# NVIDIA/tacotron2

Measured on AMD Instinct MI355X. Metric: mel-frames/sec (train fwd+bwd) LJSpeech hparams, higher is better.
Workload: dtype bf16; 1 GPU; BASELINE configs[1]: LJSpeech default hparams, batch_size=64/GPU, synthetic LJSpeech-shaped batches, full train step (fwd+loss+bwd+clip+Adam); global_batch=64, parallelism=dp1, optimizer=FusedAdam, compute=bf16 MFMA operands, f32 accumulate/state/master weights

## Files before the change

### include/tacotron2_amd.h

```cpp
#ifndef TACOTRON2_AMD_H
#define TACOTRON2_AMD_H

#include <stdint.h>

#ifdef __cplusplus
extern "C" {
#endif

#define T2AMD_ABI_VERSION 1
#define T2AMD_OK 0
#define T2AMD_ERR_ARG 1
#define T2AMD_ERR_LAUNCH 2

#define T2AMD_ATT_DIM 128
#define T2AMD_LOC_FILTERS 32
#define T2AMD_LOC_KERNEL 31
#define T2AMD_LOC_TAPS (2 * T2AMD_LOC_KERNEL)
#define T2AMD_ATT_SLICES 4

int t2amd_abi_version(void);
const char* t2amd_source_sha1(void);
const char* t2amd_last_error(void);
int t2amd_struct_sizes(int* out, int max_n);
int t2amd_set_validate_only(int on);
// ... 15 lines not shown
    long long strideSplitC;
    int accumulate;
    const float* bias;
    int act;
    const uint8_t* keep;
    long long ldkeep;
    float keep_scale;
    int convA_T, convA_C, convA_pad, convA_sign;
    int convB_T, convB_C, convB_pad;
    int precision;
} t2amd_gemm_desc;

int t2amd_gemm_tile_size(int M, int N, int precision, int nz, int a_kcontig, int b_kcontig);
int t2amd_gemm_f32(const t2amd_gemm_desc* d, void* stream);

int t2amd_splitk_reduce_f32(const float* partials, int nsplit, long long stride, float* out,
                            long long n, int accumulate, int perm_taps, int perm_ci, void* stream);
int t2amd_splitk_reduce2d_f32(const float* partials, int nsplit, long long stride, float* out, int rows, int cols,
                              long long ldo, int accumulate, void* stream);

typedef struct t2amd_gemm16_desc {
    const void* A;
    const void* B;
    float* C;
    int M, N, K;
    long long lda, ldb, ldc;
    int splitk;
    long long strideSplitC;
    int accumulate;
    const float* bias;
    int win_T, win_Tp;
} t2amd_gemm16_desc;
int t2amd_gemm16_tn(const t2amd_gemm16_desc* d, void* stream);
int t2amd_gemm16_kk(const t2amd_gemm16_desc* d, void* stream);
int t2amd_gemm16_kk_group(const t2amd_gemm16_desc* d, int count, void* stream);

int t2amd_cast_halo_bf16(const float* src, long long lds, void* dst, long long rows, int C, int T, int pad, void* stream);

int t2amd_pack_conv_bf16(const float* W, void* out, int Co, int Ci, int k, int Kp, int reversed, void* stream);

int t2amd_transpose_cast_bf16(const void* src, int src_is_bf16, long long lds, void* dst, long long ldd, int rows, int cols,
                              int rows_padded, void* stream);

int t2amd_bn_stats_f32(const float* x, long long ldx, int M, int N, double* ws, float* mean,
                       float* invstd, float* running_mean, float* running_var, float momentum,
                       float eps, void* stream);
int t2amd_bn_eval_invstd_f32(const float* running_var, float* invstd, int N, float eps, void* stream);
int t2amd_bn_act_fwd_f32(const float* x, long long ldx, float* y, long long ldy, int M, int N,
                         const float* mean, const float* invstd, const float* gamma,
                         const float* beta, int act, const uint8_t* keep, long long ldkeep,
                         float keep_scale, const int* lens, int row_valid_T, void* stream);
int t2amd_bn_act_fwd_img_f32(const float* x, long long ldx, float* y, long long ldy, int M, int N, const float* mean,
                             const float* invstd, const float* gamma, const float* beta, int act, const uint8_t* keep,
                             long long ldkeep, float keep_scale, void* y_img16, int T, int pad, void* stream);
int t2amd_bn_act_bwd_f32(float* dy, long long lddy, const float* y, long long ldy, const float* x,
                         long long ldx, int M, int N, const float* mean, const float* invstd,
                         const float* gamma, int act, const uint8_t* keep, long long ldkeep,
                         float keep_scale, double* ws, float* dgamma, float* dbeta, void* stream);
int t2amd_bn_act_bwd_img_f32(float* dy, long long lddy, const float* y, long long ldy, const float* x, long long ldx, int M, int N,
                             const float* mean, const float* invstd, const float* gamma, int act, const uint8_t* keep,
                             long long ldkeep, float keep_scale, double* ws, float* dgamma, float* dbeta, void* dx_img16, int T,
                             int pad, float* dbias, int keep_f32, void* stream);
int t2amd_colsum_f32(const float* x, long long ldx, int M, int N, double* ws, float* out,
                     int accumulate, void* stream);
int t2amd_colsum_bf16(const void* x16, long long ldx, int M, int N, double* ws, float* out, int accumulate, void* stream);

// ... 695 lines not shown
```

### tacotron2_amd/csrc/api.hip

```cpp
#include "common.h"
#include <string.h>
#include <vector>

static thread_local char g_err[512] = "";

extern "C" void t2amd_set_error_(const char* msg) {
    strncpy(g_err, msg ? msg : "", sizeof(g_err) - 1);
    g_err[sizeof(g_err) - 1] = 0;
}
extern "C" const char* t2amd_last_error(void) { return g_err; }
static int g_validate_only = 0;
extern "C" int t2amd_validate_only_flag_(void) { return g_validate_only; }
extern "C" int t2amd_set_validate_only(int on) { g_validate_only = on ? 1 : 0; return T2AMD_OK; }
extern "C" int t2amd_abi_version(void) { return T2AMD_ABI_VERSION; }
#ifndef T2AMD_SOURCE_SHA1
#define T2AMD_SOURCE_SHA1 ""
#endif
extern "C" const char* t2amd_source_sha1(void) { return T2AMD_SOURCE_SHA1; }

extern "C" int t2amd_struct_sizes(int* out, int max_n) {
    const int sizes[] = {
        (int)sizeof(t2amd_gemm_desc), (int)sizeof(t2amd_seg),       (int)sizeof(t2amd_lstm_step),
        (int)sizeof(t2amd_skinny_gemm), (int)sizeof(t2amd_addend),  (int)sizeof(t2amd_lstm_bwd),
        (int)sizeof(t2amd_attn_fwd),  (int)sizeof(t2amd_attn_bwd),  (int)sizeof(t2amd_dec_train),
        (int)sizeof(t2amd_dec_train_bwd), (int)sizeof(t2amd_lstm_seq), (int)sizeof(t2amd_dec_infer),
        (int)sizeof(t2amd_small_linear), (int)sizeof(t2amd_tensor_list), (int)sizeof(t2amd_adam_hyper),
        (int)sizeof(t2amd_dec_persist), (int)sizeof(t2amd_gemm16_desc),
    };
    const int n = (int)(sizeof(sizes) / sizeof(sizes[0]));
    for (int i = 0; i < n && i < max_n; ++i) out[i] = sizes[i];
    return n;
}

static int g_prof_tag = -1, g_prof_max = 0, g_prof_n = 0;
static std::vector<hipEvent_t> g_prof_ev;
static hipEvent_t g_cal_ev[8];
static int g_cal_have = 0, g_cal_done = 0;

extern "C" void t2amd_profile_mark_(int tag, int end, hipStream_t s) {
    if (g_prof_tag < 0 || tag != g_prof_tag || g_validate_only) return;
    if (!end) {
        if (g_prof_n >= g_prof_max) return;
        if (!g_cal_done) {
            if (!g_cal_have) {
                for (int i = 0; i < 8; ++i) (void)hipEventCreate(&g_cal_ev[i]);
                g_cal_have = 1;
// ... 518 lines not shown
```

### tacotron2_amd/csrc/common.h

```cpp
#pragma once
#include <hip/hip_runtime.h>
#include <hip/hip_ext.h>
#include <stdint.h>
#include <stdio.h>
#include "../../include/tacotron2_amd.h"

typedef float f32x4 __attribute__((ext_vector_type(4)));
typedef float f32x16 __attribute__((ext_vector_type(16)));

#define T2_WAVE 64

extern "C" void t2amd_set_error_(const char* msg);

#define T2_FAIL(msg)                                                                   \
    do {                                                                               \
        t2amd_set_error_(msg);                                                         \
        return T2AMD_ERR_ARG;                                                          \
    } while (0)

#define T2_REQUIRE(cond, msg)                                                          \
    do {                                                                               \
        if (!(cond)) T2_FAIL(msg);                                                     \
    } while (0)

extern "C" int t2amd_validate_only_flag_(void);

extern "C" void t2amd_profile_mark_(int tag, int end, hipStream_t s);

#define T2_LAUNCH(kern, grid, block, lds, stream, ...)                                 \
    do {                                                                               \
        if (!t2amd_validate_only_flag_())                                              \
            hipLaunchKernelGGL(kern, grid, block, lds, stream, __VA_ARGS__);           \
    } while (0)

extern "C" bool t2amd_profile_pair_(int tag, hipEvent_t* e0, hipEvent_t* e1);
#define T2_LAUNCH_ROLE(role, kern, grid, block, lds, stream, ...)                      \
    do {                                                                               \
        if (t2amd_validate_only_flag_()) break;                                        \
        hipEvent_t pe0_ = nullptr, pe1_ = nullptr;                                     \
        if (t2amd_profile_pair_(role, &pe0_, &pe1_))                                   \
            hipExtLaunchKernelGGL(kern, grid, block, lds, stream, pe0_, pe1_, 0, __VA_ARGS__); \
        else                                                                           \
            hipLaunchKernelGGL(kern, grid, block, lds, stream, __VA_ARGS__);           \
    } while (0)

#define T2_LAUNCH_CHECK()                                                              \
    do {                                                                               \
        if (t2amd_validate_only_flag_()) break;                                        \
        hipError_t e_ = hipGetLastError();                                             \
        if (e_ != hipSuccess) {                                                        \
            t2amd_set_error_(hipGetErrorString(e_));                                   \
            return T2AMD_ERR_LAUNCH;                                                   \
        }                                                                              \
    } while (0)

#define T2_PROPAGATE(call)                                                             \
    do {                                                                               \
        int rc_ = (call);                                                              \
// ... 158 lines not shown
```

### tacotron2_amd/csrc/gemm16.hip

```cpp
#include "common.h"
#include <stdlib.h>

typedef __bf16 g16_bf16x8 __attribute__((ext_vector_type(8)));
typedef __attribute__((address_space(3))) void* g16_lptr;
typedef __attribute__((address_space(1))) const void* g16_gptr;

#define G16_T 256
#define G16_BK 64
#define G16_IMG (G16_T * 128)
#define G16_NT 512

struct Gemm16Params {
    t2amd_gemm16_desc d;
    int ktiles_per_split;
};

struct G16Tile { int bx, by, bz; };
__device__ __forceinline__ G16Tile g16_tile_id() {
    const int nbx = gridDim.x, nby = gridDim.y;
    const int total = nbx * nby * (int)gridDim.z;
    const int L = blockIdx.x + nbx * (blockIdx.y + nby * blockIdx.z);
    const int xcd = L & 7, q = L >> 3;
    const int base = total >> 3, rem = total & 7;
    const int id = xcd * base + (xcd < rem ? xcd : rem) + q;
    const int per_z = nbx * nby;
    G16Tile t;
    t.bz = id / per_z;
    const int r = id - t.bz * per_z;
    const int G = 8;
    const int group = r / (G * nbx);
    const int first = group * G;
    const int gsz = (nby - first) < G ? (nby - first) : G;
    const int w = r - group * (G * nbx);
    t.by = first + w % gsz;
    t.bx = w / gsz;
    return t;
}

__global__ __launch_bounds__(G16_NT) void gemm16_tn_kernel(Gemm16Params p) {
    __shared__ __attribute__((aligned(16))) char smem[4 * G16_IMG];
    const t2amd_gemm16_desc& d = p.d;
    const int tid = threadIdx.x, lane = tid & 63;
    const int wave = __builtin_amdgcn_readfirstlane(tid >> 6);
    const int wm = wave >> 2, wn = wave & 3;
    const int l31 = lane & 31, lhi = lane >> 5;

    const G16Tile tile = g16_tile_id();
    const int split = tile.bz;
    const int row0 = tile.by * G16_T, col0 = tile.bx * G16_T;
    const int M = d.M, N = d.N;
    const int nkt_all = d.K / G16_BK;
    const int kt_beg = split * p.ktiles_per_split;
    int kt_end = kt_beg + p.ktiles_per_split;
    if (kt_end > nkt_all) kt_end = nkt_all;
    const int nk = kt_end > kt_beg ? kt_end - kt_beg : 0;

    const char* asrc[4];
    const char* bsrc[4];
    {
        const int rin = 8 * wave + (lane >> 3);
        const int chunk = (lane & 7) ^ ((rin >> 1) & 7);
#pragma unroll
        for (int i = 0; i < 4; ++i) {
            int ga = row0 + 64 * i + rin, gb = col0 + 64 * i + rin;
            ga = ga < M ? ga : M - 1;
            gb = gb < N ? gb : N - 1;
            asrc[i] = reinterpret_cast<const char*>(d.A) + ((long long)ga * d.lda + (long long)kt_beg * G16_BK) * 2 + chunk * 16;
            bsrc[i] = reinterpret_cast<const char*>(d.B) + ((long long)gb * d.ldb + (long long)kt_beg * G16_BK) * 2 + chunk * 16;
        }
    }
#define G16_ISSUE(STAGE)                                                                                         \
    {                                                                                                            \
        char* ad_ = smem + (STAGE) * G16_IMG + wave * 1024;                                                      \
        char* bd_ = smem + (2 + (STAGE)) * G16_IMG + wave * 1024;                                                \
        _Pragma("unroll") for (int i = 0; i < 4; ++i) {                                                          \
            __builtin_amdgcn_global_load_lds((g16_gptr)(asrc[i]), (g16_lptr)(ad_ + i * 8192), 16, 0, 0);         \
            __builtin_amdgcn_global_load_lds((g16_gptr)(bsrc[i]), (g16_lptr)(bd_ + i * 8192), 16, 0, 0);         \
            asrc[i] += 128; bsrc[i] += 128;                                                                      \
        }                                                                                                        \
    }

    unsigned aaddr[4][4], baddr[2][4];
    {
        const unsigned base = (unsigned)reinterpret_cast<size_t>((g16_lptr)(smem));
#pragma unroll
        for (int t = 0; t < 4; ++t) {
            const int r = wm * 128 + t * 32 + l31;
#pragma unroll
            for (int ks = 0; ks < 4; ++ks) aaddr[t][ks] = base + (unsigned)(r * 128 + (((2 * ks + lhi) ^ ((r >> 1) & 7)) << 4));
        }
#pragma unroll
        for (int t = 0; t < 2; ++t) {
            const int r = wn * 64 + t * 32 + l31;
#pragma unroll
            for (int ks = 0; ks < 4; ++ks)
                baddr[t][ks] = base + 2 * G16_IMG + (unsigned)(r * 128 + (((2 * ks + lhi) ^ ((r >> 1) & 7)) << 4));
        }
    }

    f32x16 acc[4][2];
#pragma unroll
    for (int i = 0; i < 4; ++i)
#pragma unroll
        for (int j = 0; j < 2; ++j)
#pragma unroll
            for (int r = 0; r < 16; ++r) acc[i][j][r] = 0.f;

    f32x4 fa[4], fb[2], ga[4], gb[2];
#define G16_READ(STAGE, KS, A_, B_)                                                                              \
    asm volatile(                                                                                                \
        "ds_read_b128 %0, %6 offset:%12\n\t"                                                                     \
        "ds_read_b128 %4, %10 offset:%12\n\t"                                                                    \
        "ds_read_b128 %1, %7 offset:%12\n\t"                                                                     \
        "ds_read_b128 %5, %11 offset:%12\n\t"                                                                    \
        "ds_read_b128 %2, %8 offset:%12\n\t"                                                                     \
        "ds_read_b128 %3, %9 offset:%12"                                                                         \
        : "=&v"(A_[0]), "=&v"(A_[1]), "=&v"(A_[2]), "=&v"(A_[3]), "=&v"(B_[0]), "=&v"(B_[1])                     \
        : "v"(aaddr[0][KS]), "v"(aaddr[1][KS]), "v"(aaddr[2][KS]), "v"(aaddr[3][KS]), "v"(baddr[0][KS]),          \
          "v"(baddr[1][KS]), "i"((STAGE) * G16_IMG)                                                              \
        : "memory");
#define G16_WAIT(A_, B_)                                                                                         \
    asm volatile("s_waitcnt lgkmcnt(0)"                                                                          \
                 : "+v"(A_[0]), "+v"(A_[1]), "+v"(A_[2]), "+v"(A_[3]), "+v"(B_[0]), "+v"(B_[1]) : : "memory");
#define G16_MFMA(A_, B_)                                                                                         \
    _Pragma("unroll") for (int i = 0; i < 4; ++i)                                                                \
        _Pragma("unroll") for (int j = 0; j < 2; ++j)                                                            \
            acc[i][j] = __builtin_amdgcn_mfma_f32_32x32x16_bf16(__builtin_bit_cast(g16_bf16x8, A_[i]),           \
                                                                __builtin_bit_cast(g16_bf16x8, B_[j]), acc[i][j], 0, 0, 0);
#define G16_TILE(STAGE)                                                                                          \
    {                                                                                                            \
        G16_READ(STAGE, 0, fa, fb) G16_WAIT(fa, fb)                                                              \
        G16_READ(STAGE, 1, ga, gb) __builtin_amdgcn_sched_barrier(0); G16_MFMA(fa, fb) __builtin_amdgcn_sched_barrier(0); G16_WAIT(ga, gb) \
        G16_READ(STAGE, 2, fa, fb) __builtin_amdgcn_sched_barrier(0); G16_MFMA(ga, gb) __builtin_amdgcn_sched_barrier(0); G16_WAIT(fa, fb) \
        G16_READ(STAGE, 3, ga, gb) __builtin_amdgcn_sched_barrier(0); G16_MFMA(fa, fb) __builtin_amdgcn_sched_barrier(0); G16_WAIT(ga, gb) \
        G16_MFMA(ga, gb)                                                                                         \
    }

    if (nk > 0) {
        G16_ISSUE(0)
        asm volatile("s_waitcnt vmcnt(0)" ::: "memory");
        __builtin_amdgcn_s_barrier();
        for (int kt = 0; kt + 1 < nk; kt += 2) {
            G16_ISSUE(1)
            G16_TILE(0)
            asm volatile("s_waitcnt vmcnt(0)" ::: "memory");
            __builtin_amdgcn_s_barrier();
            if (kt + 2 < nk) G16_ISSUE(0)
            G16_TILE(1)
            asm volatile("s_waitcnt vmcnt(0)" ::: "memory");
            __builtin_amdgcn_s_barrier();
        }
        if (nk & 1) G16_TILE(0)
    }
#undef G16_ISSUE
#undef G16_READ
#undef G16_WAIT
#undef G16_MFMA
#undef G16_TILE

    float* __restrict__ C = d.C + (long long)split * d.strideSplitC;
#pragma unroll
    for (int tm = 0; tm < 4; ++tm) {
#pragma unroll
        for (int tn = 0; tn < 2; ++tn) {
            const int gn = col0 + wn * 64 + tn * 32 + l31;
#pragma unroll
            for (int r = 0; r < 16; ++r) {
                const int gm = row0 + wm * 128 + tm * 32 + (r & 3) + 8 * (r >> 2) + 4 * lhi;
                long long crow = gm;
                bool live = gm < M;
                if (d.win_Tp > 0) {
                    const int b_ = gm / d.win_Tp, t_ = gm - b_ * d.win_Tp;
                    live = live && t_ < d.win_T;
                    crow = (long long)b_ * d.win_T + t_;
                }
                if (live && gn < N) {
                    float* cp = C + crow * d.ldc + gn;
                    float val = acc[tm][tn][r];
                    if (d.bias) val += d.bias[gn];
                    if (d.accumulate) val += *cp;
                    *cp = val;
                }
            }
        }
    }
}

extern "C" int t2amd_gemm16_tn(const t2amd_gemm16_desc* dp, void* stream) {
    T2_REQUIRE(dp != nullptr, "gemm16: null descriptor");
    Gemm16Params p;
    p.d = *dp;
    t2amd_gemm16_desc& d = p.d;
    T2_REQUIRE(d.A && d.B && d.C, "gemm16: null operand");
    T2_REQUIRE(d.M > 0 && d.N > 0 && d.K > 0 && d.K % G16_BK == 0, "gemm16: K must be a positive multiple of 64");
    T2_REQUIRE(t2_aligned16(d.A) && t2_aligned16(d.B) && d.lda % 8 == 0 && d.ldb % 8 == 0 && d.ldb >= d.K,
               "gemm16: operands must be 16-byte aligned with row strides that are multiples of 8 elements (B's >= K)");
    T2_REQUIRE(d.win_Tp == 0 || (d.win_T > 0 && d.win_T <= d.win_Tp && d.splitk == 1), "gemm16: bad window geometry");
    T2_REQUIRE(d.win_Tp > 0 || d.lda >= d.K, "gemm16: lda must be >= K unless the rows are windows");
    if (d.splitk < 1) d.splitk = 1;
    T2_REQUIRE(d.splitk == 1 || (!d.bias && !d.accumulate), "gemm16: split-K needs a plain epilogue");
    const int nkt = d.K / G16_BK;
    p.ktiles_per_split = t2_cdiv(nkt, d.splitk);
    dim3 grid(t2_cdiv(d.N, G16_T), t2_cdiv(d.M, G16_T), d.splitk);
    T2_REQUIRE(grid.y <= 65535 && grid.z <= 65535, "gemm16: grid too large");
    T2_LAUNCH(gemm16_tn_kernel, grid, dim3(G16_NT), 0, (hipStream_t)stream, p);
    T2_LAUNCH_CHECK();
    return T2AMD_OK;
}

typedef float g16_f32x2 __attribute__((ext_vector_type(2)));

#define G16_GROUP 4
struct Gemm16GroupParams {
    t2amd_gemm16_desc d[G16_GROUP];
    int coltile_end[G16_GROUP];
    int count;
};

__global__ __launch_bounds__(G16_NT) void gemm16_kk_kernel(Gemm16GroupParams p) {
    __shared__ __attribute__((aligned(16))) char smem[4 * G16_IMG];
    const int tid = threadIdx.x, lane = tid & 63;
    const int wave = __builtin_amdgcn_readfirstlane(tid >> 6);
    const int wm = wave >> 2, wn = wave & 3;
    const int l31 = lane & 31, lhi = lane >> 5;

    const G16Tile tile = g16_tile_id();
    const int split = tile.bz;
    int prob = 0;
#pragma unroll
    for (int j = 0; j + 1 < G16_GROUP; ++j)
        if (j + 1 < p.count && tile.bx >= p.coltile_end[j]) prob = j + 1;
    const int bx = tile.bx - (prob > 0 ? p.coltile_end[prob - 1] : 0);
    struct { const void* A; const void* B; float* C; int M, N, K; long long lda, ldb, ldc; long long strideSplitC; int accumulate;
             const float* bias; int splitk; } d;
    d.A = p.d[prob].A; d.B = p.d[prob].B; d.C = p.d[prob].C; d.M = p.d[prob].M; d.N = p.d[prob].N; d.K = p.d[prob].K;
    d.lda = p.d[prob].lda; d.ldb = p.d[prob].ldb; d.ldc = p.d[prob].ldc; d.strideSplitC = p.d[prob].strideSplitC;
    d.accumulate = p.d[prob].accumulate; d.bias = p.d[prob].bias; d.splitk = p.d[prob].splitk;
    const int row0 = tile.by * G16_T, col0 = bx * G16_T;
// ... 310 lines not shown
```

### tacotron2_amd/native.py

```python
import ctypes as C
import os

import torch

_HERE = os.path.dirname(os.path.abspath(__file__))
LIB_PATH = os.environ.get("T2AMD_LIB", os.path.join(_HERE, "lib", "libtacotron2_amd.so"))

TORCH_OPS_PATH = os.path.join(_HERE, "lib", "libtacotron2_amd_torch.so")

ATT_DIM = 128
LOC_FILTERS = 32
LOC_KERNEL = 31
LOC_TAPS = 62
ATT_SLICES = 4

_f32p = C.c_void_p
_i64 = C.c_longlong


class GemmDesc(C.Structure):
    _fields_ = [
        ("A", _f32p), ("B", _f32p), ("C", _f32p),
        ("M", C.c_int), ("N", C.c_int), ("K", C.c_int),
        ("lda", _i64), ("ldb", _i64), ("ldc", _i64),
# ... 195 lines not shown
class DecPersist(C.Structure):
    _fields_ = [
        ("Ti", C.c_int), ("E", C.c_int), ("H", C.c_int), ("P", C.c_int), ("C", C.c_int),
        ("max_steps", C.c_int), ("gate_threshold", C.c_float),
        ("Wa16", C.c_void_p), ("Wd16", C.c_void_p), ("bias_a", _f32p), ("bias_d", _f32p),
        ("Wq", _f32p), ("U", _f32p), ("v", _f32p), ("Wf", _f32p), ("bias_f", _f32p), ("W2", _f32p),
        ("memory", _f32p), ("pm", _f32p), ("keep_prenet", C.c_void_p),
        ("PG", _f32p), ("ALIGN", _f32p), ("out_length", C.c_void_p), ("status", C.c_void_p),
        ("steps_done", C.c_void_p), ("mailbox", C.c_void_p), ("trace", _f32p), ("timing", C.c_void_p),
        ("weights_f32", C.c_int),
    ]


PERSIST_TIMEOUT = 7
MAX_TENSORS = 64


class TensorList(C.Structure):
    _fields_ = [("param", C.c_void_p * MAX_TENSORS), ("grad", C.c_void_p * MAX_TENSORS),
                ("exp_avg", C.c_void_p * MAX_TENSORS), ("exp_avg_sq", C.c_void_p * MAX_TENSORS),
                ("numel", C.c_longlong * MAX_TENSORS), ("first_block", C.c_int * MAX_TENSORS), ("count", C.c_int)]


class AdamHyper(C.Structure):
    _fields_ = [("step_size", C.c_float), ("bc2_sqrt", C.c_float), ("one_minus_beta1", C.c_float),
                ("beta2", C.c_float), ("one_minus_beta2", C.c_float), ("eps", C.c_float), ("weight_decay", C.c_float)]


_STRUCTS = [GemmDesc, Seg, LstmStep, SkinnyGemm, Addend, LstmBwd, AttnFwd, AttnBwd, DecTrain,
            DecTrainBwd, LstmSeq, DecInfer, SmallLinear, TensorList, AdamHyper, DecPersist, Gemm16Desc]

SYMBOLS = [
    "t2amd_abi_version", "t2amd_source_sha1", "t2amd_last_error", "t2amd_struct_sizes", "t2amd_set_validate_only", "t2amd_profile_enable", "t2amd_profile_read", "t2amd_profile_event_overhead",
    "t2amd_gemm_f32", "t2amd_gemm_tile_size", "t2amd_splitk_reduce_f32", "t2amd_splitk_reduce2d_f32", "t2amd_gemm16_tn", "t2amd_gemm16_kk", "t2amd_gemm16_kk_group", "t2amd_transpose_cast_bf16", "t2amd_cast_halo_bf16", "t2amd_pack_conv_bf16",
    "t2amd_bn_stats_f32", "t2amd_bn_eval_invstd_f32", "t2amd_bn_act_fwd_f32", "t2amd_bn_act_bwd_f32", "t2amd_bn_act_bwd_img_f32", "t2amd_colsum_bf16", "t2amd_bn_act_fwd_img_f32",
    "t2amd_colsum_f32",
    "t2amd_embedding_fwd_f32", "t2amd_embedding_bwd_f32", "t2amd_philox_keep_mask", "t2amd_fill_f32",
    "t2amd_copy2d_f32", "t2amd_cast_bf16_f32", "t2amd_split_bf16x3_f32", "t2amd_transpose_f32", "t2amd_frames_to_time_major_f32",
    "t2amd_split_projection_f32", "t2amd_finalize_outputs_f32", "t2amd_grads_to_channel_last_f32",
    "t2amd_gather_dout_f32", "t2amd_relu_dropout_bwd_f32",
    "t2amd_lstm_step_fwd_f32", "t2amd_skinny_gemm_f32", "t2amd_lstm_pointwise_bwd_f32",
    "t2amd_lstm_step_fwd2_f32", "t2amd_skinny_gemm2_f32", "t2amd_lstm_pointwise_bwd2_f32",
    "t2amd_fold_location_f32", "t2amd_unfold_location_grads_f32",
    "t2amd_attention_step_fwd_f32", "t2amd_attention_step_bwd_f32",
    "t2amd_decoder_train_fwd_loop_f32", "t2amd_decoder_train_bwd_loop_f32",
    "t2amd_decoder_train_fwd_persistent_flag_bytes", "t2amd_decoder_train_fwd_persistent_supported", "t2amd_decoder_train_fwd_persistent_f32",
    "t2amd_lstm_seq_fwd_f32", "t2amd_lstm_seq_bwd_f32", "t2amd_decoder_infer_steps_f32",
    "t2amd_set_decoder_streams", "t2amd_set_bptt_cell_fold", "t2amd_get_bptt_cell_fold", "t2amd_attn_bwd_ws_floats",
    "t2amd_set_small_batch_max", "t2amd_get_small_batch_max", "t2amd_dec_infer_uses_tiles",
    "t2amd_set_attn_bwd_granules", "t2amd_attn_handoff_timeouts", "t2amd_set_attn_bwd_fused", "t2amd_attn_fwd_ws_floats", "t2amd_set_attn_fwd_fused", "t2amd_lstm_step_small_f32", "t2amd_linear_small_f32",
    "t2amd_lstm_seq_fwd2_f32", "t2amd_lstm_seq_bwd2_f32",
    "t2amd_lstm_seq_persistent_mailbox_bytes", "t2amd_lstm_seq_persistent_supported", "t2amd_lstm_seq_fwd2_persistent_f32",
    "t2amd_lstm_seq_batch_persistent_flag_bytes", "t2amd_lstm_seq_batch_persistent_supported", "t2amd_lstm_seq_fwd2_batch_persistent_f32", "t2amd_encoder_handoff_timeouts",
    "t2amd_lstm_seq_bwd2_batch_persistent_supported", "t2amd_lstm_seq_bwd2_batch_persistent_f32",
    "t2amd_reflect_pad_f32", "t2amd_reflect_index", "t2amd_stft_magnitude_f32", "t2amd_mel_log_compress_f32",
    "t2amd_mel_log_bwd_f32", "t2amd_stft_magnitude_bwd_f32", "t2amd_stft_frames_fold_f32", "t2amd_mel_l1_rows_per_slot",
    "t2amd_mel_l1_fwd_f32", "t2amd_mel_l1_bwd_f32",
    "t2amd_stft_loss_rows_per_slot", "t2amd_stft_loss_fwd_f32", "t2amd_stft_loss_finish_f64", "t2amd_stft_loss_bwd_f32",
    "t2amd_stft_loss_sum_f32",
    "t2amd_resample_plan", "t2amd_resample_fwd_f32", "t2amd_resample_bwd_f32",
    "t2amd_dtw_width", "t2amd_mel_cepstrum_f32", "t2amd_dtw_f32", "t2amd_dtw_backtrack",
    "t2amd_yin_plan", "t2amd_yin_f32",
    "t2amd_align_limits", "t2amd_align_workspace", "t2amd_monotonic_align_f32",
    "t2amd_forward_sum_workspace", "t2amd_forward_sum_f32", "t2amd_forward_sum_bwd_f32",
    "t2amd_aligner_workspace", "t2amd_aligner_pack_keys_f32", "t2amd_aligner_transpose_f32", "t2amd_aligner_rows_fwd_f32",
    "t2amd_aligner_rows_bwd_f32", "t2amd_aligner_scores_f32", "t2amd_aligner_scores_bwd_f32", "t2amd_aligner_product_f32",
    "t2amd_beta_binomial_log_prior_f32",
# ... 60 lines not shown
        "t2amd_skinny_gemm_f32": [pt(SkinnyGemm), _P],
        "t2amd_lstm_pointwise_bwd_f32": [pt(LstmBwd), _P],
        "t2amd_lstm_step_fwd2_f32": [pt(LstmStep), pt(LstmStep), _P],
        "t2amd_skinny_gemm2_f32": [pt(SkinnyGemm), pt(SkinnyGemm), _P],
        "t2amd_lstm_pointwise_bwd2_f32": [pt(LstmBwd), pt(LstmBwd), _P],
        "t2amd_fold_location_f32": [_P, _P, _P, _P],
        "t2amd_unfold_location_grads_f32": [_P, _P, _I, _P, _P, _P, _P, _P, _P],
        "t2amd_attention_step_fwd_f32": [pt(AttnFwd), _P],
        "t2amd_attention_step_bwd_f32": [pt(AttnBwd), _P],
        "t2amd_decoder_train_fwd_loop_f32": [pt(DecTrain), _P],
        "t2amd_decoder_train_fwd_persistent_flag_bytes": [_I, _I],
        "t2amd_decoder_train_fwd_persistent_supported": [pt(DecTrain), _I],
        "t2amd_decoder_train_fwd_persistent_f32": [pt(DecTrain), _P, _P, _P, _P],
        "t2amd_decoder_train_bwd_loop_f32": [pt(DecTrainBwd), _P],
        "t2amd_lstm_seq_fwd_f32": [pt(LstmSeq), _P],
        "t2amd_lstm_seq_bwd_f32": [pt(LstmSeq), _P],
        "t2amd_lstm_seq_fwd2_f32": [pt(LstmSeq), pt(LstmSeq), _P],
        "t2amd_lstm_seq_bwd2_f32": [pt(LstmSeq), pt(LstmSeq), _P],
        "t2amd_lstm_seq_persistent_mailbox_bytes": [_I, _I],
        "t2amd_lstm_seq_persistent_supported": [pt(LstmSeq)],
        "t2amd_lstm_seq_fwd2_persistent_f32": [pt(LstmSeq), pt(LstmSeq), _P, _P, _P],
        "t2amd_lstm_seq_batch_persistent_flag_bytes": [_I, _I, _I],
        "t2amd_lstm_seq_batch_persistent_supported": [pt(LstmSeq), _I, _I],
        "t2amd_lstm_seq_fwd2_batch_persistent_f32": [pt(LstmSeq), pt(LstmSeq), _P, _P, _P, _P],
        "t2amd_lstm_seq_bwd2_batch_persistent_supported": [pt(LstmSeq), _I, _I],
        "t2amd_lstm_seq_bwd2_batch_persistent_f32": [pt(LstmSeq), pt(LstmSeq), _P, _P, _P, _P],
        "t2amd_encoder_handoff_timeouts": [_I],
        "t2amd_decoder_infer_steps_f32": [pt(DecInfer), _P],
        "t2amd_struct_sizes": [pt(C.c_int), _I],
        "t2amd_set_validate_only": [_I],
        "t2amd_set_decoder_streams": [_I],
        "t2amd_set_bptt_cell_fold": [_I],
        "t2amd_get_bptt_cell_fold": [],
        "t2amd_set_small_batch_max": [_I],
        "t2amd_get_small_batch_max": [_I],
        "t2amd_dec_infer_uses_tiles": [_I, _I, _I, _I, _I, _I],
        "t2amd_attn_bwd_ws_floats": [_I, _I],
        "t2amd_set_attn_bwd_granules": [_I],
        "t2amd_attn_handoff_timeouts": [_I],
        "t2amd_set_attn_bwd_fused": [_I],
        "t2amd_attn_fwd_ws_floats": [_I, _I],
        "t2amd_set_attn_fwd_fused": [_I],
        "t2amd_lstm_step_small_f32": [pt(LstmStep), _P],
        "t2amd_linear_small_f32": [pt(SmallLinear), _P],
        "t2amd_profile_enable": [_I, _I],
        "t2amd_profile_read": [pt(C.c_float), pt(C.c_int)],
        "t2amd_profile_event_overhead": [pt(C.c_float)],
        "t2amd_reflect_pad_f32": [_P, _L, _P, _L, _I, _I, _I, _I, _P],
        "t2amd_stft_magnitude_f32": [_P, _L, _P, _L, _L, _I, _I, _P],
        "t2amd_mel_log_compress_f32": [_P, _L, _P, _I, _I, _I, _F, _P],
        "t2amd_mel_log_bwd_f32": [_P, _P, _L, _P, _L, _I, _I, _I, _F, _P],
        "t2amd_stft_magnitude_bwd_f32": [_P, _L, _P, _L, _P, _L, _L, _I, _I, _P],
        "t2amd_stft_frames_fold_f32": [_P, _L, _L, _P, _L, _L, _I, _I, _I, _I, _I, _I, _P],
        "t2amd_mel_l1_rows_per_slot": [_I],
        "t2amd_mel_l1_fwd_f32": [_P, _P, _P, _I, _I, _I, _I, _L, _P, _L, _P],
        "t2amd_mel_l1_bwd_f32": [_P, _P, _P, _P, _I, _I, _I, _I, _L, _P, _P],
        "t2amd_stft_loss_rows_per_slot": [_I],
        "t2amd_stft_loss_fwd_f32": [_P, _L, _P, _L, _P, _I, _I, _I, _F, _P, _L, _P],
        "t2amd_stft_loss_finish_f64": [_P, _L, _P, _P, _I, _F, _F, _P, _P, _P, _P],
        "t2amd_stft_loss_bwd_f32": [_P, _L, _P, _L, _P, _P, _P, _I, _I, _I, _I, _F, _P, _L, _L, _P],
        "t2amd_stft_loss_sum_f32": [_P, _L, _L, _I, _L, _P, _P],
        "t2amd_resample_plan": [_I, _I, _I, _I, pt(C.c_int), pt(C.c_int)],
        "t2amd_resample_fwd_f32": [_P, _L, _P, _I, _L, _P, _L, _L, _P, _P, _I, _I, _I, _I, _P],
        "t2amd_resample_bwd_f32": [_P, _L, _P, _I, _L, _L, _P, _L, _P, _P, _I, _I, _I, _I, _I, _P],
        "t2amd_dtw_width": [],
        "t2amd_mel_cepstrum_f32": [_P, _L, _L, _P, _I, _I, _I, _P, _I, _P, _P],
# ... 212 lines not shown
def tacotron2_loss_bwd(mel, post, tgt, gate, gate_tgt, upstream, d_mel, d_post, d_gate):
    for t in (mel, post, tgt, gate, gate_tgt, upstream, d_mel, d_post, d_gate):
        _fullc(t)
    _check(load().t2amd_tacotron2_loss_bwd_f32(ptr(mel), ptr(post), ptr(tgt), mel.numel(), ptr(gate), ptr(gate_tgt),
                                               gate.numel(), ptr(upstream), ptr(d_mel), ptr(d_post), ptr(d_gate), _stream()),
           "t2amd_tacotron2_loss_bwd_f32")


def loss_workspace_doubles():
    return int(load().t2amd_loss_workspace_doubles())


_decoder_streams = 1


def set_decoder_streams(n):
    global _decoder_streams
    _check(load().t2amd_set_decoder_streams(int(n)), "t2amd_set_decoder_streams")
    _decoder_streams = int(n)


def decoder_streams():
    return _decoder_streams


def set_bptt_cell_fold(on):
    _check(load().t2amd_set_bptt_cell_fold(1 if on else 0), "t2amd_set_bptt_cell_fold")


def get_bptt_cell_fold():
    return int(load().t2amd_get_bptt_cell_fold())


def set_small_batch_max(n):
    _check(load().t2amd_set_small_batch_max(int(n)), "t2amd_set_small_batch_max")


def small_batch_max(bf16=0):
    return int(load().t2amd_get_small_batch_max(int(bf16)))


def dec_infer_uses_tiles(B, bf16, E, Ha, Hd, P):
    return bool(load().t2amd_dec_infer_uses_tiles(int(B), int(bf16), int(E), int(Ha), int(Hd), int(P)))


def small_batch_max_setting():
    a, b = small_batch_max(0), small_batch_max(1)
    return -1 if a != b else a


def set_validate_only(on):
    global _validate_only
    load().t2amd_set_validate_only(1 if on else 0)
    _validate_only = bool(on)


def validate_only():
    return _validate_only


def profile_enable(tag, max_launches):
    _check(load().t2amd_profile_enable(tag, max_launches), "t2amd_profile_enable")


def profile_event_overhead():
    ms = C.c_float(0)
# ... 2125 lines not shown
```

Measured before the change: 649,600 valid mel-frames/s.

## Add software-pipelined gemm16 main loop interleaving LDS reads, DMA and MFMA

Adds a new main loop for the bf16 TN GEMM, on by default. It interleaves LDS fragment reads and global-to-LDS DMA issues between individual MFMA pairs, separated by sched barriers, and waits with vmcnt(8) so the next stage's loads stay in flight. Per-row source pointers become 32-bit offsets from a shared base, with a 64-bit wide variant kept for large strides, and LDS read addresses are formed by XOR with the k-step, which lowers register use. The goal is to hide LDS and global latency behind matrix math, at the cost of more barriers per tile and a more fragile hand-written schedule.

```diff
diff --git a/include/tacotron2_amd.h b/include/tacotron2_amd.h
--- a/include/tacotron2_amd.h
+++ b/include/tacotron2_amd.h
@@ -71,6 +71,8 @@
     int win_T, win_Tp;
 } t2amd_gemm16_desc;
 int t2amd_gemm16_tn(const t2amd_gemm16_desc* d, void* stream);
+int t2amd_set_gemm16_loop(int which);
+int t2amd_get_gemm16_loop(void);
 int t2amd_gemm16_kk(const t2amd_gemm16_desc* d, void* stream);
 int t2amd_gemm16_kk_group(const t2amd_gemm16_desc* d, int count, void* stream);
 
diff --git a/tacotron2_amd/csrc/api.hip b/tacotron2_amd/csrc/api.hip
--- a/tacotron2_amd/csrc/api.hip
+++ b/tacotron2_amd/csrc/api.hip
@@ -1,4 +1,5 @@
 #include "common.h"
+#include <stdlib.h>
 #include <string.h>
 #include <vector>
 
@@ -12,6 +13,14 @@
 static int g_validate_only = 0;
 extern "C" int t2amd_validate_only_flag_(void) { return g_validate_only; }
 extern "C" int t2amd_set_validate_only(int on) { g_validate_only = on ? 1 : 0; return T2AMD_OK; }
+static int g_gemm16_loop = [] { const char* e = getenv("T2AMD_GEMM16_LOOP"); return e ? (e[0] != '0') : 1; }();
+extern "C" int t2amd_gemm16_loop_flag_(void) { return g_gemm16_loop; }
+extern "C" int t2amd_set_gemm16_loop(int which) {
+    T2_REQUIRE(which == 0 || which == 1, "set_gemm16_loop: 0 or 1");
+    g_gemm16_loop = which;
+    return T2AMD_OK;
+}
+extern "C" int t2amd_get_gemm16_loop(void) { return g_gemm16_loop; }
 extern "C" int t2amd_abi_version(void) { return T2AMD_ABI_VERSION; }
 #ifndef T2AMD_SOURCE_SHA1
 #define T2AMD_SOURCE_SHA1 ""
diff --git a/tacotron2_amd/csrc/common.h b/tacotron2_amd/csrc/common.h
--- a/tacotron2_amd/csrc/common.h
+++ b/tacotron2_amd/csrc/common.h
@@ -24,6 +24,7 @@
     } while (0)
 
 extern "C" int t2amd_validate_only_flag_(void);
+extern "C" int t2amd_gemm16_loop_flag_(void);
 
 extern "C" void t2amd_profile_mark_(int tag, int end, hipStream_t s);
 
diff --git a/tacotron2_amd/csrc/gemm16.hip b/tacotron2_amd/csrc/gemm16.hip
--- a/tacotron2_amd/csrc/gemm16.hip
+++ b/tacotron2_amd/csrc/gemm16.hip
@@ -1,5 +1,6 @@
 #include "common.h"
 #include <stdlib.h>
+#include <type_traits>
 
 typedef __bf16 g16_bf16x8 __attribute__((ext_vector_type(8)));
 typedef __attribute__((address_space(3))) void* g16_lptr;
@@ -37,8 +38,9 @@
     return t;
 }
 
+template <int LOOP, bool WIDE>
 __global__ __launch_bounds__(G16_NT) void gemm16_tn_kernel(Gemm16Params p) {
-    __shared__ __attribute__((aligned(16))) char smem[4 * G16_IMG];
+    __shared__ __attribute__((aligned(128))) char smem[4 * G16_IMG];
     const t2amd_gemm16_desc& d = p.d;
     const int tid = threadIdx.x, lane = tid & 63;
     const int wave = __builtin_amdgcn_readfirstlane(tid >> 6);
@@ -55,8 +57,10 @@
     if (kt_end > nkt_all) kt_end = nkt_all;
     const int nk = kt_end > kt_beg ? kt_end - kt_beg : 0;
 
-    const char* asrc[4];
-    const char* bsrc[4];
+    typedef typename std::conditional<WIDE, unsigned long long, unsigned>::type g16_off;
+    const char* ap = reinterpret_cast<const char*>(d.A) + ((long long)row0 * d.lda + (long long)kt_beg * G16_BK) * 2;
+    const char* bp = reinterpret_cast<const char*>(d.B) + ((long long)col0 * d.ldb + (long long)kt_beg * G16_BK) * 2;
+    g16_off aoff[4], boff[4];
     {
         const int rin = 8 * wave + (lane >> 3);
         const int chunk = (lane & 7) ^ ((rin >> 1) & 7);
@@ -65,36 +69,33 @@
             int ga = row0 + 64 * i + rin, gb = col0 + 64 * i + rin;
             ga = ga < M ? ga : M - 1;
             gb = gb < N ? gb : N - 1;
-            asrc[i] = reinterpret_cast<const char*>(d.A) + ((long long)ga * d.lda + (long long)kt_beg * G16_BK) * 2 + chunk * 16;
-            bsrc[i] = reinterpret_cast<const char*>(d.B) + ((long long)gb * d.ldb + (long long)kt_beg * G16_BK) * 2 + chunk * 16;
-        }
-    }
+            aoff[i] = (g16_off)((unsigned long long)(ga - row0) * (unsigned long long)d.lda * 2 + chunk * 16);
+            boff[i] = (g16_off)((unsigned long long)(gb - col0) * (unsigned long long)d.ldb * 2 + chunk * 16);
+        }
+    }
+#define G16_DMA_A(STAGE, I, AP_)                                                                                 \
+    __builtin_amdgcn_global_load_lds((g16_gptr)((AP_) + aoff[I]), (g16_lptr)(smem + (STAGE) * G16_IMG + wave * 1024 + (I) * 8192), 16, 0, 0);
+#define G16_DMA_B(STAGE, I, BP_)                                                                                 \
+    __builtin_amdgcn_global_load_lds((g16_gptr)((BP_) + boff[I]), (g16_lptr)(smem + (2 + (STAGE)) * G16_IMG + wave * 1024 + (I) * 8192), 16, 0, 0);
 #define G16_ISSUE(STAGE)                                                                                         \
     {                                                                                                            \
-        char* ad_ = smem + (STAGE) * G16_IMG + wave * 1024;                                                      \
-        char* bd_ = smem + (2 + (STAGE)) * G16_IMG + wave * 1024;                                                \
-        _Pragma("unroll") for (int i = 0; i < 4; ++i) {                                                          \
-            __builtin_amdgcn_global_load_lds((g16_gptr)(asrc[i]), (g16_lptr)(ad_ + i * 8192), 16, 0, 0);         \
-            __builtin_amdgcn_global_load_lds((g16_gptr)(bsrc[i]), (g16_lptr)(bd_ + i * 8192), 16, 0, 0);         \
-            asrc[i] += 128; bsrc[i] += 128;                                                                      \
-        }                                                                                                        \
-    }
-
-    unsigned aaddr[4][4], baddr[2][4];
+        G16_DMA_A(STAGE, 0, ap) G16_DMA_B(STAGE, 0, bp) G16_DMA_A(STAGE, 1, ap) G16_DMA_B(STAGE, 1, bp)          \
+        G16_DMA_A(STAGE, 2, ap) G16_DMA_B(STAGE, 2, bp) G16_DMA_A(STAGE, 3, ap) G16_DMA_B(STAGE, 3, bp)          \
+        ap += 128; bp += 128;                                                                                    \
+    }
+
+    unsigned afrag[4], bfrag[2];
     {
         const unsigned base = (unsigned)reinterpret_cast<size_t>((g16_lptr)(smem));
 #pragma unroll
         for (int t = 0; t < 4; ++t) {
             const int r = wm * 128 + t * 32 + l31;
-#pragma unroll
-            for (int ks = 0; ks < 4; ++ks) aaddr[t][ks] = base + (unsigned)(r * 128 + (((2 * ks + lhi) ^ ((r >> 1) & 7)) << 4));
+            afrag[t] = base + (unsigned)(r * 128 + ((lhi ^ ((r >> 1) & 7)) << 4));
         }
 #pragma unroll
         for (int t = 0; t < 2; ++t) {
             const int r = wn * 64 + t * 32 + l31;
-#pragma unroll
-            for (int ks = 0; ks < 4; ++ks)
-                baddr[t][ks] = base + 2 * G16_IMG + (unsigned)(r * 128 + (((2 * ks + lhi) ^ ((r >> 1) & 7)) << 4));
+            bfrag[t] = base + 2 * G16_IMG + (unsigned)(r * 128 + ((lhi ^ ((r >> 1) & 7)) << 4));
         }
     }
 
@@ -107,17 +108,18 @@
             for (int r = 0; r < 16; ++r) acc[i][j][r] = 0.f;
 
     f32x4 fa[4], fb[2], ga[4], gb[2];
+    unsigned xt;
 #define G16_READ(STAGE, KS, A_, B_)                                                                              \
     asm volatile(                                                                                                \
-        "ds_read_b128 %0, %6 offset:%12\n\t"                                                                     \
-        "ds_read_b128 %4, %10 offset:%12\n\t"                                                                    \
-        "ds_read_b128 %1, %7 offset:%12\n\t"                                                                     \
-        "ds_read_b128 %5, %11 offset:%12\n\t"                                                                    \
-        "ds_read_b128 %2, %8 offset:%12\n\t"                                                                     \
-        "ds_read_b128 %3, %9 offset:%12"                                                                         \
-        : "=&v"(A_[0]), "=&v"(A_[1]), "=&v"(A_[2]), "=&v"(A_[3]), "=&v"(B_[0]), "=&v"(B_[1])                     \
-        : "v"(aaddr[0][KS]), "v"(aaddr[1][KS]), "v"(aaddr[2][KS]), "v"(aaddr[3][KS]), "v"(baddr[0][KS]),          \
-          "v"(baddr[1][KS]), "i"((STAGE) * G16_IMG)                                                              \
+        "v_xor_b32 %6, %14, %7\n\tds_read_b128 %0, %6 offset:%13\n\t"                                           \
+        "v_xor_b32 %6, %14, %11\n\tds_read_b128 %4, %6 offset:%13\n\t"                                          \
+        "v_xor_b32 %6, %14, %8\n\tds_read_b128 %1, %6 offset:%13\n\t"                                           \
+        "v_xor_b32 %6, %14, %12\n\tds_read_b128 %5, %6 offset:%13\n\t"                                          \
+        "v_xor_b32 %6, %14, %9\n\tds_read_b128 %2, %6 offset:%13\n\t"                                           \
+        "v_xor_b32 %6, %14, %10\n\tds_read_b128 %3, %6 offset:%13"                                               \
+        : "=&v"(A_[0]), "=&v"(A_[1]), "=&v"(A_[2]), "=&v"(A_[3]), "=&v"(B_[0]), "=&v"(B_[1]), "=&v"(xt)          \
+        : "v"(afrag[0]), "v"(afrag[1]), "v"(afrag[2]), "v"(afrag[3]), "v"(bfrag[0]), "v"(bfrag[1]),              \
+          "i"((STAGE) * G16_IMG), "i"(32 * (KS))                                                                 \
         : "memory");
 #define G16_WAIT(A_, B_)                                                                                         \
     asm volatile("s_waitcnt lgkmcnt(0)"                                                                          \
@@ -136,22 +138,123 @@
         G16_MFMA(ga, gb)                                                                                         \
     }
 
-    if (nk > 0) {
-        G16_ISSUE(0)
-        asm volatile("s_waitcnt vmcnt(0)" ::: "memory");
-        __builtin_amdgcn_s_barrier();
-        for (int kt = 0; kt + 1 < nk; kt += 2) {
-            G16_ISSUE(1)
-            G16_TILE(0)
+    if constexpr (LOOP == 0) {
+        if (nk > 0) {
+            G16_ISSUE(0)
             asm volatile("s_waitcnt vmcnt(0)" ::: "memory");
             __builtin_amdgcn_s_barrier();
-            if (kt + 2 < nk) G16_ISSUE(0)
-            G16_TILE(1)
-            asm volatile("s_waitcnt vmcnt(0)" ::: "memory");
+            for (int kt = 0; kt + 1 < nk; kt += 2) {
+                G16_ISSUE(1)
+                G16_TILE(0)
+                asm volatile("s_waitcnt vmcnt(0)" ::: "memory");
+                __builtin_amdgcn_s_barrier();
+                if (kt + 2 < nk) G16_ISSUE(0)
+                G16_TILE(1)
+                asm volatile("s_waitcnt vmcnt(0)" ::: "memory");
+                __builtin_amdgcn_s_barrier();
+            }
+            if (nk & 1) G16_TILE(0)
+        }
+    } else {
+        f32x4 qa0[2][4], qa1[2][4], qx[4], qy[4];
+#define G16P_RD4(D_, ADDR_, STAGE)                                                                               \
+    asm volatile("ds_read_b128 %0, %5 offset:%6\n\t"                                                             \
+                 "v_xor_b32 %4, 32, %5\n\tds_read_b128 %1, %4 offset:%6\n\t"                                    \
+                 "v_xor_b32 %4, 64, %5\n\tds_read_b128 %2, %4 offset:%6\n\t"                                    \
+                 "v_xor_b32 %4, 0x60, %5\n\tds_read_b128 %3, %4 offset:%6"                                        \
+                 : "=&v"(D_[0]), "=&v"(D_[1]), "=&v"(D_[2]), "=&v"(D_[3]), "=&v"(xt)                              \
+                 : "v"(ADDR_), "i"((STAGE) * G16_IMG)                                                            \
+                 : "memory");
+#define G16P_WAIT4(D_)                                                                                           \
+    asm volatile("s_waitcnt lgkmcnt(0)" : "+v"(D_[0]), "+v"(D_[1]), "+v"(D_[2]), "+v"(D_[3]) : : "memory");
+#define G16P_WAIT12(A_, B_)                                                                                      \
+    asm volatile("s_waitcnt lgkmcnt(0)"                                                                          \
+                 : "+v"(A_[0][0]), "+v"(A_[0][1]), "+v"(A_[0][2]), "+v"(A_[0][3]), "+v"(A_[1][0]), "+v"(A_[1][1]), \
+                   "+v"(A_[1][2]), "+v"(A_[1][3]), "+v"(B_[0]), "+v"(B_[1]), "+v"(B_[2]), "+v"(B_[3]) : : "memory");
+#define G16P_WAIT8(A_)                                                                                           \
+    asm volatile("s_waitcnt lgkmcnt(0)"                                                                          \
+                 : "+v"(A_[0][0]), "+v"(A_[0][1]), "+v"(A_[0][2]), "+v"(A_[0][3]), "+v"(A_[1][0]), "+v"(A_[1][1]), \
+                   "+v"(A_[1][2]), "+v"(A_[1][3]) : : "memory");
+#define G16P_SB __builtin_amdgcn_sched_barrier(0);
+#define G16P_MM(AH, BH, A_, B_, KS)                                                                              \
+    acc[2 * (AH)][BH] = __builtin_amdgcn_mfma_f32_32x32x16_bf16(__builtin_bit_cast(g16_bf16x8, A_[0][KS]),       \
+                                                                __builtin_bit_cast(g16_bf16x8, B_[KS]), acc[2 * (AH)][BH], 0, 0, 0); \
+    acc[2 * (AH) + 1][BH] = __builtin_amdgcn_mfma_f32_32x32x16_bf16(__builtin_bit_cast(g16_bf16x8, A_[1][KS]),   \
+                                                                    __builtin_bit_cast(g16_bf16x8, B_[KS]), acc[2 * (AH) + 1][BH], 0, 0, 0); \
+    G16P_SB
+#define G16P_STEP(STAGE, BX_, BY_, U)                                                                            \
+    {                                                                                                            \
+        const bool has1_ = (U) + 1 < nk, has2_ = (U) + 2 < nk;                                                   \
+                                                                                                    \
+        G16P_MM(0, 0, qa0, BX_, 0)                                                                               \
+        G16P_RD4(BY_, bfrag[1], STAGE) G16P_SB                                                                   \
+        G16P_MM(0, 0, qa0, BX_, 1)                                                                               \
+        if (has2_) { G16_DMA_A(STAGE, 0, ap) } G16P_SB                                                           \
+        G16P_MM(0, 0, qa0, BX_, 2)                                                                               \
+        if (has2_) { G16_DMA_A(STAGE, 2, ap) } G16P_SB                                                           \
+        G16P_MM(0, 0, qa0, BX_, 3)                                                                               \
+        G16P_WAIT4(BY_) __builtin_amdgcn_s_barrier(); G16P_SB                                                    \
+                                                                                                    \
+        G16P_MM(0, 1, qa0, BY_, 0)                                                                               \
+        G16P_RD4(qa1[0], afrag[2], STAGE) G16P_SB                                                                \
+        G16P_MM(0, 1, qa0, BY_, 1)                                                                               \
+        G16P_RD4(qa1[1], afrag[3], STAGE) G16P_SB                                                                \
+        G16P_MM(0, 1, qa0, BY_, 2)                                                                               \
+        if (has2_) { G16_DMA_B(STAGE, 0, bp) G16_DMA_B(STAGE, 1, bp) } G16P_SB                                   \
+        G16P_MM(0, 1, qa0, BY_, 3)                                                                               \
+        if (has2_) { G16_DMA_B(STAGE, 2, bp) G16_DMA_B(STAGE, 3, bp) } G16P_SB                                   \
+        G16P_WAIT8(qa1) __builtin_amdgcn_s_barrier(); G16P_SB                                                    \
+                                                                                                    \
+        G16P_MM(1, 1, qa1, BY_, 0)                                                                               \
+        if (has2_) { G16_DMA_A(STAGE, 1, ap) } G16P_SB                                                           \
+        G16P_MM(1, 1, qa1, BY_, 1)                                                                               \
+        if (has2_) { G16_DMA_A(STAGE, 3, ap) ap += 128; bp += 128; } G16P_SB                                     \
+        G16P_MM(1, 1, qa1, BY_, 2)                                                                               \
+        G16P_MM(1, 1, qa1, BY_, 3)                                                                               \
+        if (has2_) asm volatile("s_waitcnt vmcnt(8)" ::: "memory");                                              \
+        else asm volatile("s_waitcnt vmcnt(0)" ::: "memory");                                                    \
+        __builtin_amdgcn_s_barrier(); G16P_SB                                                                    \
+                                                                                                    \
+        G16P_MM(1, 0, qa1, BX_, 0)                                                                               \
+        if (has1_) { G16P_RD4(qa0[0], afrag[0], 1 - (STAGE)) } G16P_SB                                           \
+        G16P_MM(1, 0, qa1, BX_, 1)                                                                               \
+        if (has1_) { G16P_RD4(qa0[1], afrag[1], 1 - (STAGE)) } G16P_SB                                           \
+        G16P_MM(1, 0, qa1, BX_, 2)                                                                               \
+        if (has1_) { G16P_RD4(BY_, bfrag[0], 1 - (STAGE)) } G16P_SB                                              \
+        G16P_MM(1, 0, qa1, BX_, 3)                                                                               \
+        G16P_WAIT12(qa0, BY_) __builtin_amdgcn_s_barrier(); G16P_SB                                              \
+    }
+        if (nk > 0) {
+            G16_ISSUE(0)
+            if (nk > 1) {
+                G16_ISSUE(1)
+                asm volatile("s_waitcnt vmcnt(8)" ::: "memory");
+            } else {
+                asm volatile("s_waitcnt vmcnt(0)" ::: "memory");
+            }
             __builtin_amdgcn_s_barrier();
-        }
-        if (nk & 1) G16_TILE(0)
-    }
+            G16P_SB
+            G16P_RD4(qa0[0], afrag[0], 0) G16P_RD4(qa0[1], afrag[1], 0) G16P_RD4(qx, bfrag[0], 0)
+            G16P_WAIT12(qa0, qx)
+            __builtin_amdgcn_s_barrier();
+            G16P_SB
+            int u = 0;
+            for (; u + 1 < nk; u += 2) {
+                G16P_STEP(0, qx, qy, u)
+                G16P_STEP(1, qy, qx, u + 1)
+            }
+            if (nk & 1) G16P_STEP(0, qx, qy, nk - 1)
+        }
+#undef G16P_RD4
+#undef G16P_WAIT4
+#undef G16P_WAIT8
+#undef G16P_WAIT12
+#undef G16P_SB
+#undef G16P_MM
+#undef G16P_STEP
+    }
+#undef G16_DMA_A
+#undef G16_DMA_B
 #undef G16_ISSUE
 #undef G16_READ
 #undef G16_WAIT
@@ -203,7 +306,13 @@
     p.ktiles_per_split = t2_cdiv(nkt, d.splitk);
     dim3 grid(t2_cdiv(d.N, G16_T), t2_cdiv(d.M, G16_T), d.splitk);
     T2_REQUIRE(grid.y <= 65535 && grid.z <= 65535, "gemm16: grid too large");
-    T2_LAUNCH(gemm16_tn_kernel, grid, dim3(G16_NT), 0, (hipStream_t)stream, p);
+    const bool wide = d.lda >= (1ll << 23) || d.ldb >= (1ll << 23);
+    if (wide)
+        T2_LAUNCH((gemm16_tn_kernel<0, true>), grid, dim3(G16_NT), 0, (hipStream_t)stream, p);
+    else if (t2amd_gemm16_loop_flag_())
+        T2_LAUNCH((gemm16_tn_kernel<1, false>), grid, dim3(G16_NT), 0, (hipStream_t)stream, p);
+    else
+        T2_LAUNCH((gemm16_tn_kernel<0, false>), grid, dim3(G16_NT), 0, (hipStream_t)stream, p);
     T2_LAUNCH_CHECK();
     return T2AMD_OK;
 }
diff --git a/tacotron2_amd/native.py b/tacotron2_amd/native.py
--- a/tacotron2_amd/native.py
+++ b/tacotron2_amd/native.py
@@ -251,7 +251,7 @@
 
 SYMBOLS = [
     "t2amd_abi_version", "t2amd_source_sha1", "t2amd_last_error", "t2amd_struct_sizes", "t2amd_set_validate_only", "t2amd_profile_enable", "t2amd_profile_read", "t2amd_profile_event_overhead",
-    "t2amd_gemm_f32", "t2amd_gemm_tile_size", "t2amd_splitk_reduce_f32", "t2amd_splitk_reduce2d_f32", "t2amd_gemm16_tn", "t2amd_gemm16_kk", "t2amd_gemm16_kk_group", "t2amd_transpose_cast_bf16", "t2amd_cast_halo_bf16", "t2amd_pack_conv_bf16",
+    "t2amd_gemm_f32", "t2amd_gemm_tile_size", "t2amd_splitk_reduce_f32", "t2amd_splitk_reduce2d_f32", "t2amd_gemm16_tn", "t2amd_set_gemm16_loop", "t2amd_get_gemm16_loop", "t2amd_gemm16_kk", "t2amd_gemm16_kk_group", "t2amd_transpose_cast_bf16", "t2amd_cast_halo_bf16", "t2amd_pack_conv_bf16",
     "t2amd_bn_stats_f32", "t2amd_bn_eval_invstd_f32", "t2amd_bn_act_fwd_f32", "t2amd_bn_act_bwd_f32", "t2amd_bn_act_bwd_img_f32", "t2amd_colsum_bf16", "t2amd_bn_act_fwd_img_f32",
     "t2amd_colsum_f32",
     "t2amd_embedding_fwd_f32", "t2amd_embedding_bwd_f32", "t2amd_philox_keep_mask", "t2amd_fill_f32",
@@ -378,6 +378,8 @@
         "t2amd_set_decoder_streams": [_I],
         "t2amd_set_bptt_cell_fold": [_I],
         "t2amd_get_bptt_cell_fold": [],
+        "t2amd_set_gemm16_loop": [_I],
+        "t2amd_get_gemm16_loop": [],
         "t2amd_set_small_batch_max": [_I],
         "t2amd_get_small_batch_max": [_I],
         "t2amd_dec_infer_uses_tiles": [_I, _I, _I, _I, _I, _I],
@@ -656,6 +658,14 @@
     return int(load().t2amd_get_bptt_cell_fold())
 
 
+def set_gemm16_loop(which):
+    _check(load().t2amd_set_gemm16_loop(int(which)), "t2amd_set_gemm16_loop")
+
+
+def get_gemm16_loop():
+    return int(load().t2amd_get_gemm16_loop())
+
+
 def set_small_batch_max(n):
     _check(load().t2amd_set_small_batch_max(int(n)), "t2amd_set_small_batch_max")
 
```

Result: no change. 649,500 valid mel-frames/s, median of 2 (-0.0%).
